# lhwright13/Hybrid-Classical-and-Reinforcement-Learning-Aircraft-Controllers

Hardware: AMD Instinct MI355X
Metric: env-steps/sec (whole node), rate-control task, batch 65536 per GPU (higher is better)
Workload: dtype f32 compute / f64 state

## Files before the change

hybrid-classical-and-reinforcement-learning-aircraft-controllers_amd/csrc/fdyn_core.hpp:

```cpp
#pragma once
#include <hip/hip_runtime.h>
#include <stdint.h>
#include "../../include/fdyn_layout.h"
#include "philox.hpp"

namespace fdyn {

#define FD_DEV __device__ __forceinline__

template <typename T> struct M;
template <> struct M<double> {
    static FD_DEV double sin(double x) { return ::sin(x); }
    static FD_DEV double cos(double x) { return ::cos(x); }
    static FD_DEV void sincos(double x, double& s, double& c) { ::sincos(x, &s, &c); }
    static FD_DEV double tan(double x) { return ::tan(x); }
    static FD_DEV double atan2(double y, double x) { return ::atan2(y, x); }
    static FD_DEV double asin(double x) { return ::asin(x); }
    static FD_DEV double sqrt(double x) { return ::sqrt(x); }
    static FD_DEV double exp(double x) { return ::exp(x); }
    static FD_DEV double abs(double x) { return ::fabs(x); }
    static FD_DEV double copysign(double a, double y) { return __builtin_copysign(a, y); }
    static FD_DEV double rint(double x) { return ::rint(x); }
    static FD_DEV double fmod(double x, double y) { return ::fmod(x, y); }
    static FD_DEV bool finite(double x) { return ::isfinite(x); }
// ... 26 lines not shown
FD_DEV f32x2 pk_fma(f32x2 a, f32x2 b, f32x2 c) { return __builtin_elementwise_fma(a, b, c); }
FD_DEV f32x2 bc(float x) { return (f32x2){ x, x }; }
FD_DEV f32x2 lo_only(float x) { f32x2 r; r.x = x; return r; }
FD_DEV f32x2 pk_fma_bx_nhi(f32x2 a, f32x2 b, f32x2 c)
{
    f32x2 d;
    asm("v_pk_fma_f32 %0, %1, %2, %3 op_sel_hi:[1,0,1] neg_hi:[0,0,1]" : "=v"(d) : "v"(a), "v"(b), "v"(c));
    return d;
}
FD_DEV f32x2 pk_fma_ayx_bx_nlo(f32x2 a, f32x2 b, f32x2 c)
{
    f32x2 d;
    asm("v_pk_fma_f32 %0, %1, %2, %3 op_sel:[1,0,0] op_sel_hi:[0,0,1] neg_lo:[0,0,1]" : "=v"(d) : "v"(a), "v"(b), "v"(c));
    return d;
}
FD_DEV f32x2 rotate_small(f32x2 sc, float d)
{
    const float z = d * d;
    const f32x2 p1 = pk_fma(bc(z), (f32x2){ 4.1666667908e-2f, 8.3333337680e-3f }, (f32x2){ -0.5f, -1.6666667163e-1f });
    const f32x2 p2 = pk_fma(bc(z), p1, (f32x2){ 1.0f, 0.0f });
    const float sd = __builtin_fmaf(p2.y, d, d);
    return pk_fma_bx_nhi(sc, p2, sc.yx * bc(sd));
}
FD_DEV float cos_bounded(float x)
{
    const float z = x * x;
    float p = __builtin_fmaf(z, 2.4801587e-5f, -1.3888889e-3f);
    p = __builtin_fmaf(z, p, 4.1666668e-2f);
    p = __builtin_fmaf(z, p, -0.5f);
    float c = __builtin_fmaf(z, p, 1.0f);
    if (__builtin_expect(!(z <= 0.64f), 0)) { float sn; sincos(x, sn, c); }
    return c;
}
#define FD_ATAN_WIDE_LIMIT 0.7f
FD_DEV float atan_wide(float t)
{
    const float z = t * t;
    float p = __builtin_fmaf(z, 2.0541535690e-02f, -6.1546623707e-02f);
    p = __builtin_fmaf(z, p, 1.0221967846e-01f);
    p = __builtin_fmaf(z, p, -1.4136675000e-01f);
    p = __builtin_fmaf(z, p, 1.9987617433e-01f);
    p = __builtin_fmaf(z, p, -3.3332955837e-01f);
    return __builtin_fmaf(p * z, t, t);
}
#define FD_ASIN_WIDE_LIMIT 0.75f
FD_DEV float asin_wide(float x)
// ... 6 lines not shown
    p = __builtin_fmaf(z, p, 4.1755288839e-02f);
    p = __builtin_fmaf(z, p, 7.5183674693e-02f);
    p = __builtin_fmaf(z, p, 1.6666238010e-01f);
    return __builtin_fmaf(p * z, x, x);
}
FD_DEV float asin_wide_t(float t, float z)
{
    float p = __builtin_fmaf(z, 2.1202674508e-01f, -3.1944271922e-01f);
    p = __builtin_fmaf(z, p, 2.6334178448e-01f);
    p = __builtin_fmaf(z, p, -7.6388612390e-02f);
    p = __builtin_fmaf(z, p, 5.3024884313e-02f);
    p = __builtin_fmaf(z, p, 4.1755288839e-02f);
    p = __builtin_fmaf(z, p, 7.5183674693e-02f);
    p = __builtin_fmaf(z, p, 1.6666238010e-01f);
    return __builtin_fmaf(p * z, t, t);
}
FD_DEV f32x2 atan_asin_wide(float ta, float za, float tb, float zb)
{
    const float pa = __builtin_fmaf(za, 2.0541535690e-02f, -6.1546623707e-02f);
    float pb = __builtin_fmaf(zb, 2.1202674508e-01f, -3.1944271922e-01f);
    pb = __builtin_fmaf(zb, pb, 2.6334178448e-01f);
    pb = __builtin_fmaf(zb, pb, -7.6388612390e-02f);
    const f32x2 z = { za, zb }, t = { ta, tb };
    f32x2 p = pk_fma(z, (f32x2){ pa, pb }, (f32x2){ 1.0221967846e-01f, 5.3024884313e-02f });
    p = pk_fma(z, p, (f32x2){ -1.4136675000e-01f, 4.1755288839e-02f });
    p = pk_fma(z, p, (f32x2){ 1.9987617433e-01f, 7.5183674693e-02f });
    p = pk_fma(z, p, (f32x2){ -3.3332955837e-01f, 1.6666238010e-01f });
    return pk_fma(p * z, t, t);
}
FD_DEV float atan_pos(float a)
{
    const bool big = a > 2.414213562373095f, mid = a > 0.4142135623730950f;
    const float num = big ? -1.0f : (mid ? a - 1.0f : a);
    const float den = big ? a : (mid ? a + 1.0f : 1.0f);
    const float base = big ? 1.5707963267948966f : (mid ? 0.7853981633974483f : 0.0f);
    const float t = num * rcp(den);
    const float z = t * t;
    float p = __builtin_fmaf(z, 8.05374449538e-2f, -1.38776856032e-1f);
    p = __builtin_fmaf(z, p, 1.99777106478e-1f);
    p = __builtin_fmaf(z, p, -3.33329491539e-1f);
    return base + __builtin_fmaf(p * z, t, t);
}
FD_DEV float atan2(float y, float x)
{
    const float ax = __builtin_fabsf(x), ay = __builtin_fabsf(y);
    const float mx = __builtin_fmaxf(ax, ay), mn = __builtin_fminf(ax, ay);
// ... 137 lines not shown
        derive_lane_from<FAST>(lane, src[derive_source(lane < FD_ND_LANES ? lane : 0)], blk);
    }
    template <bool FAST>
    static FD_DEV void derive_lane_from(int lane, double a, double* blk)
    {
        if (lane < 5) {
            const int to = lane == 0 ? FD_PD_INV_MASS : (lane == 1 ? FD_PD_INV_IXX : (lane == 2 ? FD_PD_INV_IYY : (lane == 3 ? FD_PD_INV_IZZ : FD_PD_INV_THRUST_ZERO_V)));
            blk[to] = 1.0 / a;
        } else if (FAST && lane < FD_ND_LANES) {
            const bool is_alpha = lane == 5;
            float snf, csf;
            fast::sincos(float(a), snf, csf);
            const double sn = snf, cs = csf;
            blk[is_alpha ? FD_PD_SIN_MAX_ALPHA : FD_PD_SIN_MAX_PITCH] = sn;
            blk[is_alpha ? FD_PD_COS_MAX_ALPHA : FD_PD_COS_MAX_PITCH] = cs;
            if (is_alpha) {
                const double tl = sn / cs;
                const bool poly_ok = a > 0.0 && a < 1.5 && tl <= double(FD_ATAN_WIDE_LIMIT);
                blk[FD_PD_TAN_ALPHA_FAST] = poly_ok ? tl : 0.0;
                blk[FD_PD_ALPHA_NEEDS_ATAN2] = poly_ok ? 0.0 : 1.0;
            }
        }
    }
};

template <typename S> struct Limits {
    S max_vel, max_rate, max_pitch, min_dt, max_dt;
    FD_DEV void load(const double* blk)
    {
        max_vel = S(blk[FD_P_MAX_VELOCITY]); max_rate = S(blk[FD_P_MAX_RATE_RAD]);
        max_pitch = S(blk[FD_P_MAX_PITCH_RAD]); min_dt = S(blk[FD_P_MIN_TIMESTEP]); max_dt = S(blk[FD_P_MAX_TIMESTEP]);
    }
};

template <typename T> struct Controls {
    T de_rad, da_rad, dr_rad, throttle;
    T cl0_de, cm_de, cl_da, cn_dr, cy, thrust_max;
    fast::f32x2 pk_da_dr;
    template <typename S> FD_DEV void set(const Params<T>& P, S elevator, S aileron, S rudder, S thr)
    {
        de_rad = T(clipv<S>(elevator, S(-1), S(1))) * P.max_de;
        da_rad = T(clipv<S>(aileron, S(-1), S(1))) * P.max_da;
        dr_rad = T(clipv<S>(rudder, S(-1), S(1))) * P.max_dr;
        throttle = T(clipv<S>(thr, S(0), S(1)));
        if constexpr (sizeof(T) == 4) {
            cl0_de = P.cl_0 + P.cl_de * de_rad;
// ... 122 lines not shown
struct Trig { fast::f32x2 phi, th, psi; };
FD_DEV Trig trig_of(float phi, float theta, float psi)
{
    Trig t;
    float s, c;
    fast::sincos(phi, s, c); t.phi = (fast::f32x2){ s, c };
    fast::sincos(theta, s, c); t.th = (fast::f32x2){ s, c };
    fast::sincos(psi, s, c); t.psi = (fast::f32x2){ s, c };
    return t;
}
FD_DEV float trig_rotate(const Trig& t0, float dphi, float dth, float dpsi, Trig& t)
{
    t.phi = fast::rotate_small(t0.phi, dphi);
    t.th = fast::rotate_small(t0.th, dth);
    t.psi = fast::rotate_small(t0.psi, dpsi);
    return __builtin_fmaxf(__builtin_fmaxf(__builtin_fabsf(dphi), __builtin_fabsf(dth)), __builtin_fabsf(dpsi));
}
FD_DEV float trig_rotate_scaled(const Trig& t0, float h, float kphi, float kth, float kpsi, Trig& t)
{
    const fast::f32x2 d2 = fast::bc(h) * (fast::f32x2){ kphi, kth };
    return trig_rotate(t0, d2.x, d2.y, h * kpsi, t);
}

#define FD_UNLIKELY(c) __builtin_expect(!!(c), 0)
#ifdef FD_PHASE_STAMPS
__device__ unsigned fdyn_dbg_cnt[4096 * 8];
#define FD_DBG_COUNT(SLOT) if (threadIdx.x < 64) { const unsigned long long m_ = __ballot(1); \
    if (int(threadIdx.x) == __ffsll((long long)m_) - 1) atomicAdd(&fdyn_dbg_cnt[blockIdx.x * 8 + (SLOT)], 1u); \
    atomicAdd(&fdyn_dbg_cnt[blockIdx.x * 8 + (SLOT) + 1], 1u); }
#define FD_DBG_COUNT1(SLOT) if (threadIdx.x < 64) atomicAdd(&fdyn_dbg_cnt[blockIdx.x * 8 + (SLOT)], 1u);
#else
#define FD_DBG_COUNT(SLOT)
#define FD_DBG_COUNT1(SLOT)
#endif

template <bool STRAIGHT = true, bool WIND = false>
FD_DEV void dynamics_fast(const Params<float>& P, const Controls<float>& C, const float (&x)[FD_NX], Trig& tg, float dmax,
                          float (&xd)[FD_NX], const Wind<float>& wnd = Wind<float>{})
{
    const float ug = x[3], vg = x[4], wg = x[5], theta = x[7];
    const float p = x[9], q = x[10], r = x[11];
    float u = ug, v = vg, w = wg;
    if constexpr (WIND) {
        if (FD_UNLIKELY(!(dmax <= 0.125f))) { tg = trig_of(x[6], theta, x[8]); dmax = 0.0f; }
        float bu, bv, bw;
        body_wind<float>(tg.phi.x, tg.phi.y, tg.th.x, tg.th.y, tg.psi.x, tg.psi.y, wnd, bu, bv, bw);
        u = ug - bu; v = vg - bv; w = wg - bw;
    }

    const fast::f32x2 vw = { v, w };
    const fast::f32x2 vw_sq = vw * vw;
    const float uw2 = __builtin_fmaf(u, u, vw_sq.y);
    const float V2 = __builtin_fmaf(v, v, uw2);
    const float airspeed = fast::sqrt(V2);
    const float Vs = fast::max_nc(airspeed, P.min_airspeed);
    const float inv_V = fast::rcp(Vs);

    const float au = __builtin_fabsf(u);
    const float au_min = fast::max_nc(au, P.min_u);
    const float us = au > 1e-6f ? __builtin_copysignf(au_min, u) : P.min_u;
    const float inv_h = fast::rsq(__builtin_fmaf(us, us, vw_sq.y));
    const fast::f32x2 xt_ab = vw * (fast::f32x2){ inv_V, fast::rcp(us) };
    const fast::f32x2 xt_sq = xt_ab * xt_ab;
    const float t_alpha = xt_ab.y;
    const bool a_in = __builtin_fabsf(w) <= P.tan_alpha_fast * us;
    const float sin_alpha = a_in ? w * inv_h : __builtin_copysignf(P.sin_max_alpha, w);
    const float cos_alpha = a_in ? us * inv_h : P.cos_max_alpha;

    const float av = __builtin_fabsf(v);
    const bool b_in = av <= FD_ASIN_WIDE_LIMIT * Vs;
    const float xb = xt_ab.x;
    auto beta_tail = [&]() {
        const float vv_rest = airspeed >= P.min_airspeed ? uw2 : __builtin_fmaxf(__builtin_fmaf(Vs, Vs, -(v * v)), 0.0f);
        const float half_om = 0.5f * (vv_rest * fast::rcp(Vs * (Vs + av)));
        const float b_r = fast::asin_wide_t(fast::sqrt(half_om), half_om);
        return __builtin_copysignf(__builtin_fmaf(-2.0f, b_r, 1.5707963267948966f), v);
    };
    float beta, b_t, z_b;
    if constexpr (STRAIGHT) {
        const float vv_rest = airspeed >= P.min_airspeed ? uw2 : __builtin_fmaxf(__builtin_fmaf(Vs, Vs, -vw_sq.x), 0.0f);
        const float half_om = 0.5f * (vv_rest * fast::rcp(Vs * (Vs + av)));
        b_t = b_in ? xb : fast::sqrt(half_om);
        z_b = b_in ? xt_sq.x : half_om;
    } else {
        b_t = xb; z_b = xt_sq.x;
    }
    const fast::f32x2 ab = fast::atan_asin_wide(t_alpha, xt_sq.y, b_t, z_b);
    const float alpha_poly = fast::pinned(ab.x);
    const float alpha = a_in ? alpha_poly : __builtin_copysignf(P.max_alpha, w);
    if constexpr (STRAIGHT) beta = b_in ? ab.y : __builtin_copysignf(__builtin_fmaf(-2.0f, ab.y, 1.5707963267948966f), v);
    else beta = ab.y;

    const bool th_in = __builtin_fabsf(theta) <= P.max_pitch;
    float sth_e = th_in ? tg.th.x : __builtin_copysignf(P.sin_max_pitch, theta);
    float cth_e = th_in ? tg.th.y : P.cos_max_pitch;

    const bool ordinary = (dmax <= 0.125f) & (P.alpha_needs_atan2 == 0.0f) & (STRAIGHT | b_in);
    float alpha_r = alpha, sin_alpha_r = sin_alpha, cos_alpha_r = cos_alpha;
    if (FD_UNLIKELY(!ordinary)) {
        FD_DBG_COUNT(0)
        if (!(dmax <= 0.125f)) {
            FD_DBG_COUNT1(4)
            tg = trig_of(x[6], theta, x[8]);
            sth_e = th_in ? tg.th.x : sth_e; cth_e = th_in ? tg.th.y : cth_e;
        }
        if (P.alpha_needs_atan2 != 0.0f) {
            const float a_raw = fast::atan2(w, us);
            const bool hi = a_raw > P.max_alpha, lo = a_raw < -P.max_alpha;
            sin_alpha_r = hi ? P.sin_max_alpha : (lo ? -P.sin_max_alpha : w * inv_h);
            cos_alpha_r = (hi || lo) ? P.cos_max_alpha : us * inv_h;
            alpha_r = clipf(a_raw, -P.max_alpha, P.max_alpha);
        }
        if constexpr (!STRAIGHT) {
            if (!b_in) beta = beta_tail();
        }
    }
    const float sth = tg.th.x, cth = tg.th.y;

    using fast::f32x2;
    using fast::bc;
    const float q_S = P.half_rho_S * V2;
    const float cl = __builtin_fmaf(P.cl_alpha, alpha_r, C.cl0_de);
    const float cd = __builtin_fmaf(P.cd_alpha2, alpha_r * alpha_r, P.cd_0);
    const f32x2 ld = bc(q_S) * (f32x2){ cl, cd };
    const f32x2 cs_a = { cos_alpha_r, sin_alpha_r };
    const f32x2 fxz = fast::pk_fma_ayx_bx_nlo(cs_a, ld, ld.yy * cs_a);
    const float thrust = C.thrust_max * __builtin_fmaxf(0.0f, __builtin_fmaf(-airspeed, P.inv_thrust_zero_v, 1.0f));

    const f32x2 g_cs = bc(P.g) * (tg.phi * bc(cth));
    xd[3] = __builtin_fmaf(fxz.x + thrust, P.inv_mass, __builtin_fmaf(r, vg, __builtin_fmaf(-q, wg, -(P.g * sth))));
    xd[4] = __builtin_fmaf(q_S * C.cy, P.inv_mass, __builtin_fmaf(p, wg, __builtin_fmaf(-r, ug, g_cs.x)));
    xd[5] = __builtin_fmaf(-fxz.y, P.inv_mass, __builtin_fmaf(q, ug, __builtin_fmaf(-p, vg, g_cs.y)));

    const f32x2 hV = P.pk_half_b_c * bc(inv_V);
    const f32x2 qSbc = bc(q_S) * P.pk_b_c;
    const f32x2 pr = { p, r };
    const f32x2 ln_in = fast::pk_fma(P.pk_damp_pr * pr, bc(hV.x), C.pk_da_dr);
    const f32x2 ln = bc(qSbc.x) * fast::pk_fma(P.pk_beta_ln, bc(beta), ln_in);
    const float m_moment = qSbc.y * __builtin_fmaf(P.cm_alpha, alpha_r, __builtin_fmaf(P.damp_pitch * q, hV.y, C.cm_de));
    const f32x2 gy = { __builtin_fmaf(-P.izz_m_iyy * q, r, ln.x), __builtin_fmaf(-P.iyy_m_ixx * p, q, ln.y) };
    const f32x2 a_pr = gy * P.pk_inv_i_pr;
    xd[9] = a_pr.x;
    xd[10] = __builtin_fmaf(-P.ixx_m_izz * p, r, m_moment) * P.inv_iyy;
    xd[11] = a_pr.y;

    const fast::f32x2 sb = fast::pk_fma_bx_nhi(tg.phi, fast::lo_only(vg), tg.phi.yx * fast::bc(wg));
    const float sv_cw = sb.x;
    const float ah = __builtin_fmaf(cth, ug, sth * sv_cw);
    const fast::f32x2 ne = fast::pk_fma_ayx_bx_nlo(tg.psi, fast::lo_only(ah), tg.psi * fast::bc(sb.y));
    xd[0] = ne.x;
    xd[1] = ne.y;
    xd[2] = __builtin_fmaf(cth, sv_cw, -(sth * ug));

    const float inv_c = fast::rcp(cth_e);
    const fast::f32x2 qt = fast::pk_fma_bx_nhi(tg.phi, fast::lo_only(q), tg.phi.yx * fast::bc(r));
    const float qr = qt.x;
    xd[8] = qr * inv_c;
    xd[6] = __builtin_fmaf(sth_e * inv_c, qr, p);
    xd[7] = qt.y;

#pragma unroll
    for (int i = 9; i < 12; ++i) xd[i] = clipf(xd[i], -P.max_ang_acc, P.max_ang_acc);
// ... 20 lines not shown
        const S v = x[i];
        x[i] = (v != v) ? S(0) : (M<S>::finite(v) ? v : (v > S(0) ? S(10000) : S(-10000)));
    }
#pragma unroll
    for (int i = 3; i < 6; ++i) x[i] = clipv(x[i], -Lm.max_vel, Lm.max_vel);
    x[6] = wrap_state_angle<S, T>(x[6]);
    x[7] = clipv(x[7], -Lm.max_pitch, Lm.max_pitch);
    x[8] = wrap_state_angle<S, T>(x[8]);
#pragma unroll
    for (int i = 9; i < 12; ++i) x[i] = clipv(x[i], -Lm.max_rate, Lm.max_rate);
    if (-x[2] < S(0)) {
        x[2] = S(0);
        x[5] = x[5] > S(0) ? x[5] : S(0);
    }
    S accs = x[0];
#pragma unroll
    for (int i = 1; i < 12; ++i) accs += x[i];
    if (!M<S>::finite(accs)) {
#pragma unroll
        for (int i = 0; i < 12; ++i) x[i] = M<S>::finite(x[i]) ? x[i] : S(0);
    }
}

struct FastRK {
    float x0[FD_NX];
    Trig t0;
    float d0;
    template <typename S> FD_DEV void init(const S (&x)[FD_NX])
    {
#pragma unroll
        for (int i = 0; i < 12; ++i) x0[i] = float(x[i]);
        t0 = trig_of(x0[6], x0[7], x0[8]);
        d0 = 0.0f;
    }
    FD_DEV void ensure_trig()
    {
        if (FD_UNLIKELY(!(d0 <= 0.125f))) { t0 = trig_of(x0[6], x0[7], x0[8]); d0 = 0.0f; }
    }
};

template <typename S, bool STRAIGHT = true, bool WIND = false>
FD_DEV void rk4_fast_step(const Params<float>& P, const Limits<S>& Lm, const Controls<float>& C, S (&x)[FD_NX], FastRK& f,
                          float hdt, float fdt, float dt6, const Wind<float>& wnd = Wind<float>{})
{
    using T = float;
    T xt[FD_NX], k[FD_NX];
    Trig tt;
    using fast::f32x2;
    constexpr int PA[6] = { 0, 2, 4, 6, 8, 10 }, PB[6] = { 1, 3, 5, 7, 9, 11 };
    f32x2 acc2[6], x02[6];
#pragma unroll
    for (int j = 0; j < 6; ++j) x02[j] = (f32x2){ f.x0[PA[j]], f.x0[PB[j]] };
    auto stage = [&](T h, T wgt, bool first) {
#pragma unroll
        for (int j = 0; j < 6; ++j) {
            const f32x2 kj = { k[PA[j]], k[PB[j]] };
            acc2[j] = first ? kj : fast::pk_fma(fast::bc(wgt), kj, acc2[j]);
            if (j >= 1) {
                const f32x2 xj = fast::pk_fma(fast::bc(h), kj, x02[j]);
                xt[PA[j]] = xj.x; xt[PB[j]] = xj.y;
            }
        }
    };
    dynamics_fast<STRAIGHT, WIND>(P, C, f.x0, f.t0, f.d0, k, wnd);
    stage(hdt, T(1), true);
    T dm = trig_rotate_scaled(f.t0, hdt, k[6], k[7], k[8], tt);
    dynamics_fast<STRAIGHT, WIND>(P, C, xt, tt, dm, k, wnd);
    stage(hdt, T(2), false);
    dm = trig_rotate_scaled(f.t0, hdt, k[6], k[7], k[8], tt);
    dynamics_fast<STRAIGHT, WIND>(P, C, xt, tt, dm, k, wnd);
    stage(fdt, T(2), false);
    dm = trig_rotate_scaled(f.t0, fdt, k[6], k[7], k[8], tt);
    dynamics_fast<STRAIGHT, WIND>(P, C, xt, tt, dm, k, wnd);
    T ksum[FD_NX], inc[FD_NX];
#pragma unroll
    for (int j = 0; j < 6; ++j) {
        const f32x2 ks = acc2[j] + (f32x2){ k[PA[j]], k[PB[j]] };
        const f32x2 in2 = fast::bc(dt6) * ks;
        ksum[PA[j]] = ks.x; ksum[PB[j]] = ks.y;
        inc[PA[j]] = in2.x; inc[PB[j]] = in2.y;
    }
#pragma unroll
    for (int i = 0; i < 12; ++i) {
        if constexpr (sizeof(S) == 4) x[i] = __builtin_fmaf(dt6, ksum[i], x[i]);
        else x[i] += S(inc[i]);
        if (STRAIGHT && i >= 9) x[i] = M<S>::abs(x[i]) > Lm.max_rate ? M<S>::copysign(Lm.max_rate, x[i]) : x[i];
        f.x0[i] = T(x[i]);
    }
    f.d0 = trig_rotate(f.t0, inc[6], inc[7], inc[8], f.t0);
    f32x2 sum2 = { f.x0[0], f.x0[1] };
#pragma unroll
    for (int j = 1; j < 6; ++j) sum2 += (f32x2){ f.x0[2 * j], f.x0[2 * j + 1] };
    const T sum = sum2.x + sum2.y;
    const T vmax = __builtin_fmaxf(__builtin_fmaxf(__builtin_fabsf(f.x0[3]), __builtin_fabsf(f.x0[4])), __builtin_fabsf(f.x0[5]));
    const T amax = __builtin_fmaxf(__builtin_fabsf(f.x0[6]), __builtin_fabsf(f.x0[8]));
    bool lim = !(vmax <= T(Lm.max_vel)) | (f.x0[2] > T(0)) | !(amax <= T(FD_PI));
    if constexpr (!STRAIGHT) {
        lim |= (M<S>::abs(x[9]) > Lm.max_rate) | (M<S>::abs(x[10]) > Lm.max_rate) | (M<S>::abs(x[11]) > Lm.max_rate);
    }
    const bool ang = !(__builtin_fabsf(f.x0[7]) <= T(Lm.max_pitch)) | !M<T>::finite(sum);
    if (FD_UNLIKELY(lim | ang)) {
        FD_DBG_COUNT(2)
#ifdef FD_PHASE_STAMPS
        if (!(vmax <= T(Lm.max_vel))) { FD_DBG_COUNT1(5) }
        if (f.x0[2] > T(0)) { FD_DBG_COUNT1(7) }
#endif
        if (ang) {
            post_step<S, T>(Lm, x);
#pragma unroll
            for (int i = 0; i < 12; ++i) f.x0[i] = T(x[i]);
            f.d0 = T(1);
        } else {
#pragma unroll
            for (int i = 3; i < 6; ++i) x[i] = clipv(x[i], -Lm.max_vel, Lm.max_vel);
            if constexpr (!STRAIGHT) {
#pragma unroll
                for (int i = 9; i < 12; ++i) {
                    x[i] = M<S>::abs(x[i]) > Lm.max_rate ? M<S>::copysign(Lm.max_rate, x[i]) : x[i];
                    f.x0[i] = T(x[i]);
                }
            }
            x[6] = wrap_state_angle<S, T>(x[6]);
            x[8] = wrap_state_angle<S, T>(x[8]);
            if (-x[2] < S(0)) {
                x[2] = S(0);
                x[5] = x[5] > S(0) ? x[5] : S(0);
            }
            f.x0[2] = T(x[2]); f.x0[6] = T(x[6]); f.x0[8] = T(x[8]);
#pragma unroll
            for (int i = 3; i < 6; ++i) f.x0[i] = T(x[i]);
        }
    }
}

template <typename S, typename T, bool STRAIGHT = true, bool WIND = false>
FD_DEV void rk4_substeps(const Params<T>& P, const Limits<S>& Lm, const Controls<T>& C, S (&x)[FD_NX], S dt, int n_sub,
                         const Wind<T>& wnd = Wind<T>{})
{
    if constexpr (sizeof(T) == 8) {
        for (int s = 0; s < n_sub; ++s) {
            T xt[FD_NX], k[FD_NX];
            S acc[FD_NX];
            const T hdt = T(S(0.5) * dt), fdt = T(dt);
#pragma unroll
            for (int i = 0; i < 12; ++i) xt[i] = T(x[i]);
            dynamics<T, WIND>(P, C, xt, k, wnd);
#pragma unroll
            for (int i = 0; i < 12; ++i) { acc[i] = S(k[i]); xt[i] = T(x[i] + S(hdt) * S(k[i])); }
            dynamics<T, WIND>(P, C, xt, k, wnd);
#pragma unroll
            for (int i = 0; i < 12; ++i) { acc[i] += S(2) * S(k[i]); xt[i] = T(x[i] + S(hdt) * S(k[i])); }
            dynamics<T, WIND>(P, C, xt, k, wnd);
#pragma unroll
            for (int i = 0; i < 12; ++i) { acc[i] += S(2) * S(k[i]); xt[i] = T(x[i] + S(fdt) * S(k[i])); }
            dynamics<T, WIND>(P, C, xt, k, wnd);
            const S dt6 = dt / S(6);
#pragma unroll
            for (int i = 0; i < 12; ++i) x[i] = x[i] + dt6 * (acc[i] + S(k[i]));
            post_step<S, T>(Lm, x);
        }
    } else {
        FastRK f;
        f.init(x);
        const T hdt = T(S(0.5) * dt), fdt = T(dt), dt6 = T(dt / S(6));
        for (int s = 0; s < n_sub; ++s) rk4_fast_step<S, STRAIGHT, WIND>(P, Lm, C, x, f, hdt, fdt, dt6, wnd);
    }
}

template <typename S> struct Derived { S airspeed, altitude, ground_speed, heading; };
template <typename S> FD_DEV Derived<S> derived(const S (&x)[FD_NX])
{
    Derived<S> d;
    const S u = x[3], v = x[4], w = x[5];
    S sphi, cphi, sth, cth, spsi, cpsi;
    M<S>::sincos(x[6], sphi, cphi);
    M<S>::sincos(x[7], sth, cth);
    M<S>::sincos(x[8], spsi, cpsi);
    d.airspeed = M<S>::sqrt(u * u + v * v + w * w);
    d.altitude = -x[2];
    const S vn = (cth * cpsi) * u + (sphi * sth * cpsi - cphi * spsi) * v + (cphi * sth * cpsi + sphi * spsi) * w;
    const S ve = (cth * spsi) * u + (sphi * sth * spsi + cphi * cpsi) * v + (cphi * sth * spsi - sphi * cpsi) * w;
    d.heading = M<S>::atan2(ve, vn);
    d.ground_speed = M<S>::sqrt(vn * vn + ve * ve);
    return d;
}
FD_DEV Derived<float> derived_fast(FastRK& f)
{
    f.ensure_trig();
// ... 301 lines not shown
```

hybrid-classical-and-reinforcement-learning-aircraft-controllers_amd/csrc/fdyn_kernels.hip:

```cpp
#include <hip/hip_runtime.h>
#include <stdint.h>
#include <math.h>
#include <string.h>
#include <stdlib.h>
#include "fdyn_fleet.hpp"

using namespace fdyn;

#define FD_BLOCK 256

struct StagedParamWords { double v0, v1, d; };
__device__ __forceinline__ StagedParamWords stage_params_early(const double* __restrict__ params, int n_types)
{
    StagedParamWords w;
    const int i0 = threadIdx.x, i1 = FD_BLOCK + threadIdx.x;
    const int t0 = i0 / FD_NP_USED, t1 = i1 / FD_NP_USED;
    w.v0 = i0 < n_types * FD_NP_USED ? params[t0 * FD_NP + (i0 - t0 * FD_NP_USED)] : 0.0;
    w.v1 = i1 < n_types * FD_NP_USED ? params[t1 * FD_NP + (i1 - t1 * FD_NP_USED)] : 0.0;
    constexpr int NDL = Params<double>::FD_ND_LANES;
    const int t = threadIdx.x / NDL;
    w.d = int(threadIdx.x) < n_types * NDL ? params[t * FD_NP + Params<double>::derive_source(threadIdx.x - t * NDL)] : 1.0;
    return w;
}
template <bool FAST>
// ... 812 lines not shown
                     const double* __restrict__ pool, int pool_depth, uint64_t seed, int auto_reset, float residual_scale,
                     float* __restrict__ obs_out , float* __restrict__ reward_f32, S* __restrict__ reward_full,
                     uint8_t* __restrict__ terminated, uint8_t* __restrict__ truncated,
                     int32_t* __restrict__ ev_count, int32_t* __restrict__ ev_count_next, int32_t* __restrict__ ev_int,
                     float* __restrict__ ev_flt, int ev_cap, int64_t n, DRA... dra)
{
    constexpr bool DR = sizeof...(DRA) != 0;
    S* dr = nullptr;
    const double* drc = nullptr;
    if constexpr (DR) dr_unpack(dr, drc, dra...);
    __shared__ double s_params[FD_MAX_TYPES * FD_NP_STAGED];
    __shared__ __attribute__((aligned(16))) float s_tile[FD_BLOCK / FD_WAVE][FD_WAVE * (FD_OBS_DIM + 1)];
    __shared__ float s_pid_cfg[3 * FD_NPC];
    __shared__ S s_consts[FD_NC];
    FD_STAMP(0)
    FD_STAMP_REAL(7)
    const LaneMap lm = lane_map(n);
    const int64_t i = lm.i;
    const int lane = lm.lane, wave = threadIdx.x / FD_WAVE;
    const bool active = lm.on;
    EnvConsts<S> ec;
    load_env_consts<S, PREP>(EC, ec);
    const bool uses_sched = ec.cmd_type == FD_CMD_RAMP || ec.cmd_type == FD_CMD_SINE;
    const bool residual_mode = actions != nullptr && residual_scale > 0.0f && pid_state != nullptr;
    const bool pid_mode = actions == nullptr || residual_mode;

    using E = typename EnvOf<S, T>::type;
    S x[FD_NX];
    EnvState<E> e;
    int32_t step = 0, episode = 0;
    int ty = 0;
    float4 av = make_float4(0.0f, 0.0f, 0.0f, 0.0f);
    S rec_pre[FD_NR];
    S wair[3] = { S(0), S(0), S(0) }, dsc[5] = { S(1), S(1), S(1), S(1), S(1) };
    const bool pre_drawn = !OCC2 && pool == nullptr && auto_reset != 0;
    constexpr bool EARLY_PARAMS = sizeof(T) == 4;
    StagedParamWords spw = { 0.0, 0.0, 1.0 };
    if constexpr (EARLY_PARAMS) spw = PREP ? stage_image_early(params, n_types) : stage_params_early(params, n_types);
    if (active) {
        episode = eis[FD_EI_EPISODE * n + i];
#pragma unroll
        for (int k = 3; k < FD_NX; ++k) x[k] = xs[k * n + i];
        if (actions) av = reinterpret_cast<const float4*>(actions)[i];
        ty = lane_type(type, i, n_types);
#pragma unroll
        for (int k = 0; k < 3; ++k) x[k] = xs[k * n + i];
// ... 57 lines not shown
#pragma unroll
                for (int k = 0; k < 4; ++k) {
                    const float c = a_in[k] + rr[k] * residual_scale;
                    const float lo = k < 3 ? -1.0f : 0.0f;
                    a_in[k] = c < lo ? lo : (c > 1.0f ? 1.0f : c);
                }
                const float mag = rr[0] * rr[0] + (rr[1] * rr[1] + rr[2] * rr[2]);
                res_bonus = S(0.05) * (S(1) - S(mag) / S(3));
            }
        }
        if (actions_out) reinterpret_cast<float4*>(actions_out)[i] = make_float4(a_in[0], a_in[1], a_in[2], a_in[3]);
        S a[4];
        a[0] = clipv(S(a_in[0]), S(-1), S(1)); a[1] = clipv(S(a_in[1]), S(-1), S(1));
        a[2] = clipv(S(a_in[2]), S(-1), S(1)); a[3] = clipv(S(a_in[3]), S(0), S(1));

        Controls<T> C;
        C.set(P, a[1], a[0], a[2], a[3]);
        const S dt_sub = ec.dt / S(ec.n_sub);
#ifdef FD_PHASE_STAMPS
        asm volatile("s_waitcnt vmcnt(0) lgkmcnt(0)" ::: "memory");
#endif
        FD_STAMP(1)
        if constexpr (DR) rk4_substeps<S, T, !OCC2, true>(P, Lm, C, x, dt_sub, ec.n_sub, Wind<T>{ T(wair[0]), T(wair[1]), T(wair[2]) });
        else rk4_substeps<S, T, !OCC2>(P, Lm, C, x, dt_sub, ec.n_sub);
        FD_STAMP(2)
        if constexpr (sizeof(E) == sizeof(S)) e.time += E(ec.dt);
        else e.time = E(S(step + 1) * ec.dt);
        step += 1;

        if (ec.cmd_type == FD_CMD_RAMP) {
            const S t = S(e.time);
            if (t < S(3)) {
                const S alpha = t / S(3);
#pragma unroll
                for (int k = 0; k < 3; ++k) e.cmd[k] = E((S(1) - alpha) * S(0) + alpha * S(e.sched[k]));
            } else {
#pragma unroll
                for (int k = 0; k < 3; ++k) e.cmd[k] = e.sched[k];
            }
        } else if (ec.cmd_type == FD_CMD_RANDOM_WALK) {
            S delta[3];
            if (rw_delta) {
#pragma unroll
                for (int k = 0; k < 3; ++k) delta[k] = rw_delta[k * n + i];
            } else {
                Philox ph; uint32_t r[4];
                ph.block(seed, uint32_t(i), uint32_t(episode), uint32_t(step), FD_PHX_RANDOM_WALK, r);
// ... 101 lines not shown
            const int leader = __ffsll((long long)done_mask) - 1;
            base = __shfl(base, leader, FD_WAVE);
            const int local = base + prefix;
            if (done && local < cap_s) {
                const int slot = shard * cap_s + local;
                ev_int[slot * FD_EV_NI + FD_EV_ENV] = int32_t(i);
                ev_int[slot * FD_EV_NI + FD_EV_LENGTH] = len_term;
                ev_int[slot * FD_EV_NI + FD_EV_TERMINATED] = term ? 1 : 0;
                ev_flt[slot * FD_EV_NF] = ret_term;
#pragma unroll
                for (int k = 0; k < FD_OBS_DIM; ++k) ev_flt[slot * FD_EV_NF + 1 + k] = o_term[k];
            }
        }
    }
    FD_STAMP(4)
    store_obs_tile(s_tile[wave], o, lane, obs_out, lm.wave_first, n);
    FD_STAMP(5)
#ifdef FD_PHASE_STAMPS
    asm volatile("s_waitcnt vmcnt(0)" ::: "memory");
#endif
    FD_STAMP_REAL(6)
}

static_assert(FD_NIMG == FD_IMG_PARAMS + FD_MAX_TYPES * FD_NP_STAGED && FD_ECD_INTS + 2 <= FD_IMG_PARAMS, "fdyn_layout.h: image sections");
template <bool FAST>
__global__ void __launch_bounds__(FD_BLOCK)
rate_env_image_kernel(const double* __restrict__ params, int n_types, const double* __restrict__ EC, double* __restrict__ image)
{
    double* blocks = image + FD_IMG_PARAMS;
    for (int i = threadIdx.x; i < FD_MAX_TYPES * FD_NP_STAGED; i += blockDim.x) {
        const int t = i / FD_NP_STAGED, k = i - t * FD_NP_STAGED;
        blocks[i] = (t < n_types && k < FD_NP_USED) ? params[t * FD_NP + k] : 0.0;
    }
    for (int k = threadIdx.x; k < FD_IMG_PARAMS; k += blockDim.x) if (k < FD_ECD_INTS || k >= FD_ECD_INTS + 2) image[FD_IMG_EC + k] = k < FD_NEC ? EC[k] : 0.0;
    __syncthreads();
    constexpr int NDL = Params<double>::FD_ND_LANES;
    if (int(threadIdx.x) < n_types * NDL) {
        const int t = threadIdx.x / NDL;
        Params<double>::derive_lane<FAST>(threadIdx.x - t * NDL, params + t * FD_NP, blocks + t * FD_NP_STAGED);
    }
    if (threadIdx.x == FD_BLOCK - 1) {
        EnvConsts<double> ec;
        load_env_consts<double>(EC, ec);
        int32_t* ic = reinterpret_cast<int32_t*>(image + FD_IMG_EC + FD_ECD_INTS);
        ic[0] = ec.max_steps; ic[1] = ec.cmd_type; ic[2] = ec.n_sub; ic[3] = ec.settle_steps;
    }
}

static int g_simds = 0;
static int simd_count()
{
    if (!g_simds) {
        int dev = 0; hipDeviceProp_t p;
        g_simds = (hipGetDevice(&dev) == hipSuccess && hipGetDeviceProperties(&p, dev) == hipSuccess) ? p.multiProcessorCount * 4 : 1024;
    }
    return g_simds;
}

#define FD_ENV_RESET_PARAMS(S, E)                                                                            \
    S* x, E* e, int32_t* ei, float* pid_state, const uint8_t* mask, const double* env_consts, const double* pool, \
    int pool_depth, uint64_t seed, float* obs_out, int64_t n
#define FD_ENV_RESET_ARGS x, e, ei, pid_state, mask, env_consts, pool, pool_depth, seed, obs_out, n
#define FD_ENV_STEP_PARAMS(S, E)                                                                             \
    S* x, E* e, int32_t* ei, const uint8_t* type, const double* params, int n_types, const double* env_consts, \
    const float* actions, float* pid_state, const float* pid_cfg, const double* casc_consts, float* actions_out, \
    const S* rw_delta, const double* pool, int pool_depth, uint64_t seed, int auto_reset, float residual_scale, \
    float* obs_out, float* reward_f32, S* reward_full, uint8_t* terminated, uint8_t* truncated, int32_t* ev_count, \
    int32_t* ev_count_next, int32_t* ev_int, float* ev_flt, int ev_cap, int64_t n
// ... 193 lines not shown
```

include/fdyn_layout.h:

```cpp
#ifndef FDYN_LAYOUT_H
#define FDYN_LAYOUT_H

enum {
    FD_X_N = 0, FD_X_E, FD_X_D,
    FD_X_U, FD_X_V, FD_X_W,
    FD_X_ROLL, FD_X_PITCH, FD_X_YAW,
    FD_X_P, FD_X_Q, FD_X_R,
    FD_NX = 12
};

enum { FD_U_ELEVATOR = 0, FD_U_AILERON, FD_U_RUDDER, FD_U_THROTTLE, FD_NU = 4 };

enum { FD_D_AIRSPEED = 0, FD_D_ALTITUDE, FD_D_GROUND_SPEED, FD_D_HEADING, FD_ND = 4 };

enum {
    FD_P_MASS = 0, FD_P_IXX, FD_P_IYY, FD_P_IZZ,
    FD_P_WING_AREA, FD_P_WING_SPAN, FD_P_CHORD,
    FD_P_CL_0, FD_P_CL_ALPHA, FD_P_CD_0, FD_P_CD_ALPHA2,
    FD_P_CL_ELEVATOR, FD_P_CM_ELEVATOR, FD_P_CY_RUDDER, FD_P_CN_RUDDER, FD_P_CL_AILERON,
    FD_P_CM_ALPHA, FD_P_CN_BETA, FD_P_CL_BETA,
    FD_P_DAMPING_ROLL, FD_P_DAMPING_PITCH, FD_P_DAMPING_YAW,
    FD_P_MAX_THRUST, FD_P_AIR_DENSITY, FD_P_GRAVITY,
    FD_P_MIN_AIRSPEED_AERO, FD_P_MIN_U_VELOCITY,
    FD_P_MAX_ELEVATOR_RAD, FD_P_MAX_AILERON_RAD, FD_P_MAX_RUDDER_RAD,
// ... 44 lines not shown
enum { FD_CMD_STEP = 0, FD_CMD_RAMP = 1, FD_CMD_SINE = 2, FD_CMD_RANDOM_WALK = 3 };

enum {
    FD_E_CMD_P = 0, FD_E_CMD_Q, FD_E_CMD_R,
    FD_E_PREV_AIL, FD_E_PREV_ELEV, FD_E_PREV_RUD, FD_E_PREV_THR,
    FD_E_PERR_P, FD_E_PERR_Q, FD_E_PERR_R,
    FD_E_SIGN_P, FD_E_SIGN_Q, FD_E_SIGN_R,
    FD_E_SETTLE_TIMER, FD_E_IS_SETTLED,
    FD_E_TIME,
    FD_E_SCHED0, FD_E_SCHED1, FD_E_SCHED2,
    FD_E_SCHED3,
    FD_E_EP_RETURN,
    FD_NE = 21
};
enum { FD_EI_STEP = 0, FD_EI_EPISODE, FD_NEI = 2 };

enum {
    FD_EC_DT = 0, FD_EC_DT_PHYSICS, FD_EC_MAX_STEPS, FD_EC_CMD_TYPE, FD_EC_DIFFICULTY_SCALE,
    FD_EC_MAX_RATE_P, FD_EC_MAX_RATE_Q, FD_EC_MAX_RATE_R,
    FD_NEC = 8
};

enum {
    FD_ECD_INTS = FD_NEC,
    FD_IMG_EC = 0, FD_IMG_PARAMS = 16,
    FD_NIMG = FD_IMG_PARAMS + 8 * FD_NP_STAGED
};

enum {
    FD_R_AIRSPEED = 0, FD_R_ALTITUDE, FD_R_ROLL, FD_R_PITCH, FD_R_YAW, FD_R_P, FD_R_Q, FD_R_R,
    FD_R_CMD0, FD_R_CMD1, FD_R_CMD2,
    FD_R_CMD3,
    FD_NR = 12
};

enum { FD_EV_ENV = 0, FD_EV_LENGTH, FD_EV_TERMINATED, FD_EV_NI = 3 };
#define FD_EV_NF (1 + FD_OBS_DIM)
enum { FD_EV_SHARDS = 64 };

enum {
    FD_DR_WIND_N = 0, FD_DR_WIND_E, FD_DR_WIND_D,
    FD_DR_GUST_N, FD_DR_GUST_E, FD_DR_GUST_D,
    FD_DR_GUST_A, FD_DR_GUST_B,
    FD_DR_MASS_S, FD_DR_IXX_S, FD_DR_IYY_S, FD_DR_IZZ_S, FD_DR_RHO_S,
    FD_NDR = 13
};
enum {
// ... 92 lines not shown
```

Before: 1.779 billion.

## Add branch-free RK4 fast path when step-size bounds prove rare cases impossible

Computes, when the parameter image is built, an a priori bound on Euler-angle increments per substep. If every aircraft type satisfies it and the alpha polynomial is valid, a flag is stored in the image. The rate kernel then ballots whether any lane is outside the rate/pitch limits and, if none are, runs an RK4 variant with the rare-case checks (dmax, atan2 fallback, pinned values) compiled out. That variant also packs the trig rotation and damping arithmetic into paired f32 ops and keeps predicate literals in scalar registers. It adds a second instantiation of the substep loop, which costs code size and register pressure, and its correctness depends on the analytic bound holding.

Measured after the change: 1.871 billion, median of 6. 5.2% higher.

```diff
diff --git a/hybrid-classical-and-reinforcement-learning-aircraft-controllers_amd/csrc/fdyn_core.hpp b/hybrid-classical-and-reinforcement-learning-aircraft-controllers_amd/csrc/fdyn_core.hpp
--- a/hybrid-classical-and-reinforcement-learning-aircraft-controllers_amd/csrc/fdyn_core.hpp
+++ b/hybrid-classical-and-reinforcement-learning-aircraft-controllers_amd/csrc/fdyn_core.hpp
@@ -72,6 +72,14 @@
     const float sd = __builtin_fmaf(p2.y, d, d);
     return pk_fma_bx_nhi(sc, p2, sc.yx * bc(sd));
 }
+FD_DEV f32x2 rotate_small_bc(f32x2 sc, f32x2 dd)
+{
+    const float z = dd.x * dd.x;
+    const f32x2 p1 = pk_fma(bc(z), (f32x2){ 4.1666667908e-2f, 8.3333337680e-3f }, (f32x2){ -0.5f, -1.6666667163e-1f });
+    const f32x2 p2 = pk_fma(bc(z), p1, (f32x2){ 1.0f, 0.0f });
+    const f32x2 sd = pk_fma(p2.yy, dd, dd);
+    return pk_fma_bx_nhi(sc, p2, sc.yx * sd);
+}
 FD_DEV float cos_bounded(float x)
 {
     const float z = x * x;
@@ -124,6 +132,18 @@
     pb = __builtin_fmaf(zb, pb, 2.6334178448e-01f);
     pb = __builtin_fmaf(zb, pb, -7.6388612390e-02f);
     const f32x2 z = { za, zb }, t = { ta, tb };
+    f32x2 p = pk_fma(z, (f32x2){ pa, pb }, (f32x2){ 1.0221967846e-01f, 5.3024884313e-02f });
+    p = pk_fma(z, p, (f32x2){ -1.4136675000e-01f, 4.1755288839e-02f });
+    p = pk_fma(z, p, (f32x2){ 1.9987617433e-01f, 7.5183674693e-02f });
+    p = pk_fma(z, p, (f32x2){ -3.3332955837e-01f, 1.6666238010e-01f });
+    return pk_fma(p * z, t, t);
+}
+FD_DEV f32x2 atan_asin_wide(f32x2 t, f32x2 z)
+{
+    const float pa = __builtin_fmaf(z.x, 2.0541535690e-02f, -6.1546623707e-02f);
+    float pb = __builtin_fmaf(z.y, 2.1202674508e-01f, -3.1944271922e-01f);
+    pb = __builtin_fmaf(z.y, pb, 2.6334178448e-01f);
+    pb = __builtin_fmaf(z.y, pb, -7.6388612390e-02f);
     f32x2 p = pk_fma(z, (f32x2){ pa, pb }, (f32x2){ 1.0221967846e-01f, 5.3024884313e-02f });
     p = pk_fma(z, p, (f32x2){ -1.4136675000e-01f, 4.1755288839e-02f });
     p = pk_fma(z, p, (f32x2){ 1.9987617433e-01f, 7.5183674693e-02f });
@@ -307,6 +327,16 @@
             }
         }
     }
+    static FD_DEV double euler_increment_bound(const double* __restrict__ src, double h)
+    {
+        constexpr double SLACK = 1.0 + 1.0 / 512.0;
+        const double R = src[FD_P_MAX_RATE_RAD], A = src[FD_P_MAX_ANGULAR_ACCELERATION], mp = src[FD_P_MAX_PITCH_RAD];
+        if (!(R >= 0.0 && A >= 0.0 && h > 0.0 && mp >= 0.0 && mp <= 1.5)) return 1.0e300;
+        const double rt2 = 1.4142135623730951;
+        const double G = fmax(1.0 + rt2 * tan(mp), rt2 / cos(mp));
+        return SLACK * h * G * (R + 0.5 * h * A);
+    }
+    static FD_DEV bool small_steps_ok(const double* __restrict__ src, double h) { return euler_increment_bound(src, h) <= 0.125; }
 };
 
 template <typename S> struct Limits {
@@ -475,6 +505,13 @@
     return trig_rotate(t0, d2.x, d2.y, h * kpsi, t);
 }
 
+FD_DEV void trig_rotate_pairs(const Trig& t0, fast::f32x2 d2, fast::f32x2 dpsi, Trig& t)
+{
+    t.phi = fast::rotate_small_bc(t0.phi, d2.xx);
+    t.th = fast::rotate_small_bc(t0.th, d2.yy);
+    t.psi = fast::rotate_small_bc(t0.psi, dpsi.xx);
+}
+
 #define FD_UNLIKELY(c) __builtin_expect(!!(c), 0)
 #ifdef FD_PHASE_STAMPS
 __device__ unsigned fdyn_dbg_cnt[4096 * 8];
@@ -487,10 +524,11 @@
 #define FD_DBG_COUNT1(SLOT)
 #endif
 
-template <bool STRAIGHT = true, bool WIND = false>
+template <bool STRAIGHT = true, bool WIND = false, bool RARE = true>
 FD_DEV void dynamics_fast(const Params<float>& P, const Controls<float>& C, const float (&x)[FD_NX], Trig& tg, float dmax,
                           float (&xd)[FD_NX], const Wind<float>& wnd = Wind<float>{})
 {
+    static_assert(RARE || (STRAIGHT && !WIND), "the block-free form exists for the straight, still-air evaluation only");
     const float ug = x[3], vg = x[4], wg = x[5], theta = x[7];
     const float p = x[9], q = x[10], r = x[11];
     float u = ug, v = vg, w = wg;
@@ -513,16 +551,23 @@
     const float au_min = fast::max_nc(au, P.min_u);
     const float us = au > 1e-6f ? __builtin_copysignf(au_min, u) : P.min_u;
     const float inv_h = fast::rsq(__builtin_fmaf(us, us, vw_sq.y));
-    const fast::f32x2 xt_ab = vw * (fast::f32x2){ inv_V, fast::rcp(us) };
+    constexpr int IA = RARE ? 1 : 0, IB = 1 - IA;
+    fast::f32x2 xt_ab, rcps = { 0.0f, 0.0f };
+    if constexpr (RARE) xt_ab = vw * (fast::f32x2){ inv_V, fast::rcp(us) };
+    else {
+        rcps = (fast::f32x2){ fast::rcp(us), inv_V };
+        asm("" : "+v"(rcps));
+        xt_ab = vw.yx * rcps;
+    }
     const fast::f32x2 xt_sq = xt_ab * xt_ab;
-    const float t_alpha = xt_ab.y;
+    const float t_alpha = xt_ab[IA];
     const bool a_in = __builtin_fabsf(w) <= P.tan_alpha_fast * us;
     const float sin_alpha = a_in ? w * inv_h : __builtin_copysignf(P.sin_max_alpha, w);
     const float cos_alpha = a_in ? us * inv_h : P.cos_max_alpha;
 
     const float av = __builtin_fabsf(v);
     const bool b_in = av <= FD_ASIN_WIDE_LIMIT * Vs;
-    const float xb = xt_ab.x;
+    const float xb = xt_ab[IB];
     auto beta_tail = [&]() {
         const float vv_rest = airspeed >= P.min_airspeed ? uw2 : __builtin_fmaxf(__builtin_fmaf(Vs, Vs, -(v * v)), 0.0f);
         const float half_om = 0.5f * (vv_rest * fast::rcp(Vs * (Vs + av)));
@@ -534,12 +579,20 @@
         const float vv_rest = airspeed >= P.min_airspeed ? uw2 : __builtin_fmaxf(__builtin_fmaf(Vs, Vs, -vw_sq.x), 0.0f);
         const float half_om = 0.5f * (vv_rest * fast::rcp(Vs * (Vs + av)));
         b_t = b_in ? xb : fast::sqrt(half_om);
-        z_b = b_in ? xt_sq.x : half_om;
+        z_b = b_in ? xt_sq[IB] : half_om;
     } else {
-        b_t = xb; z_b = xt_sq.x;
-    }
-    const fast::f32x2 ab = fast::atan_asin_wide(t_alpha, xt_sq.y, b_t, z_b);
-    const float alpha_poly = fast::pinned(ab.x);
+        b_t = xb; z_b = xt_sq[IB];
+    }
+    fast::f32x2 ab;
+    if constexpr (RARE) {
+        ab = fast::atan_asin_wide(t_alpha, xt_sq[IA], b_t, z_b);
+    } else {
+        fast::f32x2 t2 = xt_ab, z2 = xt_sq;
+        t2.y = b_t; z2.y = z_b;
+        ab = fast::atan_asin_wide(t2, z2);
+    }
+    float alpha_poly = ab.x;
+    if constexpr (RARE) alpha_poly = fast::pinned(ab.x);
     const float alpha = a_in ? alpha_poly : __builtin_copysignf(P.max_alpha, w);
     if constexpr (STRAIGHT) beta = b_in ? ab.y : __builtin_copysignf(__builtin_fmaf(-2.0f, ab.y, 1.5707963267948966f), v);
     else beta = ab.y;
@@ -548,7 +601,7 @@
     float sth_e = th_in ? tg.th.x : __builtin_copysignf(P.sin_max_pitch, theta);
     float cth_e = th_in ? tg.th.y : P.cos_max_pitch;
 
-    const bool ordinary = (dmax <= 0.125f) & (P.alpha_needs_atan2 == 0.0f) & (STRAIGHT | b_in);
+    const bool ordinary = RARE ? (dmax <= 0.125f) & (P.alpha_needs_atan2 == 0.0f) & (STRAIGHT | b_in) : true;
     float alpha_r = alpha, sin_alpha_r = sin_alpha, cos_alpha_r = cos_alpha;
     if (FD_UNLIKELY(!ordinary)) {
         FD_DBG_COUNT(0)
@@ -580,17 +633,30 @@
     const f32x2 fxz = fast::pk_fma_ayx_bx_nlo(cs_a, ld, ld.yy * cs_a);
     const float thrust = C.thrust_max * __builtin_fmaxf(0.0f, __builtin_fmaf(-airspeed, P.inv_thrust_zero_v, 1.0f));
 
-    const f32x2 g_cs = bc(P.g) * (tg.phi * bc(cth));
+    f32x2 g_cs;
+    if constexpr (RARE) g_cs = bc(P.g) * (tg.phi * bc(cth));
+    else g_cs = bc(P.g) * (tg.phi * tg.th.yy);
     xd[3] = __builtin_fmaf(fxz.x + thrust, P.inv_mass, __builtin_fmaf(r, vg, __builtin_fmaf(-q, wg, -(P.g * sth))));
     xd[4] = __builtin_fmaf(q_S * C.cy, P.inv_mass, __builtin_fmaf(p, wg, __builtin_fmaf(-r, ug, g_cs.x)));
     xd[5] = __builtin_fmaf(-fxz.y, P.inv_mass, __builtin_fmaf(q, ug, __builtin_fmaf(-p, vg, g_cs.y)));
 
-    const f32x2 hV = P.pk_half_b_c * bc(inv_V);
+    f32x2 hV;
+    if constexpr (RARE) hV = P.pk_half_b_c * bc(inv_V);
+    else hV = P.pk_half_b_c * rcps.yy;
     const f32x2 qSbc = bc(q_S) * P.pk_b_c;
-    const f32x2 pr = { p, r };
-    const f32x2 ln_in = fast::pk_fma(P.pk_damp_pr * pr, bc(hV.x), C.pk_da_dr);
+    f32x2 ln_in;
+    float damp_q = 0.0f;
+    if constexpr (RARE) {
+        const f32x2 pr = { p, r };
+        ln_in = fast::pk_fma(P.pk_damp_pr * pr, bc(hV.x), C.pk_da_dr);
+    } else {
+        const f32x2 d_qr = (f32x2){ P.damp_pitch, P.pk_damp_pr.y } * (f32x2){ q, r };
+        ln_in = (f32x2){ __builtin_fmaf(P.pk_damp_pr.x * p, hV.x, C.pk_da_dr.x), __builtin_fmaf(d_qr.y, hV.x, C.pk_da_dr.y) };
+        damp_q = d_qr.x;
+    }
     const f32x2 ln = bc(qSbc.x) * fast::pk_fma(P.pk_beta_ln, bc(beta), ln_in);
-    const float m_moment = qSbc.y * __builtin_fmaf(P.cm_alpha, alpha_r, __builtin_fmaf(P.damp_pitch * q, hV.y, C.cm_de));
+    if constexpr (RARE) damp_q = P.damp_pitch * q;
+    const float m_moment = qSbc.y * __builtin_fmaf(P.cm_alpha, alpha_r, __builtin_fmaf(damp_q, hV.y, C.cm_de));
     const f32x2 gy = { __builtin_fmaf(-P.izz_m_iyy * q, r, ln.x), __builtin_fmaf(-P.iyy_m_ixx * p, q, ln.y) };
     const f32x2 a_pr = gy * P.pk_inv_i_pr;
     xd[9] = a_pr.x;
@@ -657,10 +723,13 @@
     }
 }
 
+struct PredLits { float pi, inf, zero; };
 struct FastRK {
     float x0[FD_NX];
     Trig t0;
     float d0;
+    fast::f32x2 xp[FD_NX / 2];
+    PredLits lit;
     template <typename S> FD_DEV void init(const S (&x)[FD_NX])
     {
 #pragma unroll
@@ -674,11 +743,19 @@
     }
 };
 
-template <typename S, bool STRAIGHT = true, bool WIND = false>
+template <typename S, bool STRAIGHT = true, bool WIND = false, bool RARE = true>
 FD_DEV void rk4_fast_step(const Params<float>& P, const Limits<S>& Lm, const Controls<float>& C, S (&x)[FD_NX], FastRK& f,
                           float hdt, float fdt, float dt6, const Wind<float>& wnd = Wind<float>{})
 {
     using T = float;
+    if constexpr (!RARE) {
+#pragma unroll
+        for (int j = 0; j < 6; ++j) {
+            fast::f32x2 v = f.xp[j];
+            asm("" : "+v"(v));
+            f.x0[2 * j] = v.x; f.x0[2 * j + 1] = v.y;
+        }
+    }
     T xt[FD_NX], k[FD_NX];
     Trig tt;
     using fast::f32x2;
@@ -697,16 +774,23 @@
             }
         }
     };
-    dynamics_fast<STRAIGHT, WIND>(P, C, f.x0, f.t0, f.d0, k, wnd);
+    dynamics_fast<STRAIGHT, WIND, RARE>(P, C, f.x0, f.t0, f.d0, k, wnd);
     stage(hdt, T(1), true);
-    T dm = trig_rotate_scaled(f.t0, hdt, k[6], k[7], k[8], tt);
-    dynamics_fast<STRAIGHT, WIND>(P, C, xt, tt, dm, k, wnd);
+    auto rotate_stage = [&](T h) {
+        trig_rotate_pairs(f.t0, fast::bc(h) * (f32x2){ k[6], k[7] }, fast::bc(h) * (f32x2){ k[8], k[9] }, tt);
+    };
+    T dm = T(0);
+    if constexpr (RARE) dm = trig_rotate_scaled(f.t0, hdt, k[6], k[7], k[8], tt);
+    else rotate_stage(hdt);
+    dynamics_fast<STRAIGHT, WIND, RARE>(P, C, xt, tt, dm, k, wnd);
     stage(hdt, T(2), false);
-    dm = trig_rotate_scaled(f.t0, hdt, k[6], k[7], k[8], tt);
-    dynamics_fast<STRAIGHT, WIND>(P, C, xt, tt, dm, k, wnd);
+    if constexpr (RARE) dm = trig_rotate_scaled(f.t0, hdt, k[6], k[7], k[8], tt);
+    else rotate_stage(hdt);
+    dynamics_fast<STRAIGHT, WIND, RARE>(P, C, xt, tt, dm, k, wnd);
     stage(fdt, T(2), false);
-    dm = trig_rotate_scaled(f.t0, fdt, k[6], k[7], k[8], tt);
-    dynamics_fast<STRAIGHT, WIND>(P, C, xt, tt, dm, k, wnd);
+    if constexpr (RARE) dm = trig_rotate_scaled(f.t0, fdt, k[6], k[7], k[8], tt);
+    else rotate_stage(fdt);
+    dynamics_fast<STRAIGHT, WIND, RARE>(P, C, xt, tt, dm, k, wnd);
     T ksum[FD_NX], inc[FD_NX];
 #pragma unroll
     for (int j = 0; j < 6; ++j) {
@@ -722,18 +806,23 @@
         if (STRAIGHT && i >= 9) x[i] = M<S>::abs(x[i]) > Lm.max_rate ? M<S>::copysign(Lm.max_rate, x[i]) : x[i];
         f.x0[i] = T(x[i]);
     }
-    f.d0 = trig_rotate(f.t0, inc[6], inc[7], inc[8], f.t0);
+    if constexpr (RARE) f.d0 = trig_rotate(f.t0, inc[6], inc[7], inc[8], f.t0);
+    else trig_rotate_pairs(f.t0, (f32x2){ inc[6], inc[7] }, (f32x2){ inc[8], inc[9] }, f.t0);
     f32x2 sum2 = { f.x0[0], f.x0[1] };
 #pragma unroll
     for (int j = 1; j < 6; ++j) sum2 += (f32x2){ f.x0[2 * j], f.x0[2 * j + 1] };
     const T sum = sum2.x + sum2.y;
     const T vmax = __builtin_fmaxf(__builtin_fmaxf(__builtin_fabsf(f.x0[3]), __builtin_fabsf(f.x0[4])), __builtin_fabsf(f.x0[5]));
     const T amax = __builtin_fmaxf(__builtin_fabsf(f.x0[6]), __builtin_fabsf(f.x0[8]));
-    bool lim = !(vmax <= T(Lm.max_vel)) | (f.x0[2] > T(0)) | !(amax <= T(FD_PI));
+    bool lim;
+    if constexpr (RARE) lim = !(vmax <= T(Lm.max_vel)) | (f.x0[2] > T(0)) | !(amax <= T(FD_PI));
+    else lim = !(vmax <= T(Lm.max_vel)) | (f.x0[2] > f.lit.zero) | !(amax <= f.lit.pi);
     if constexpr (!STRAIGHT) {
         lim |= (M<S>::abs(x[9]) > Lm.max_rate) | (M<S>::abs(x[10]) > Lm.max_rate) | (M<S>::abs(x[11]) > Lm.max_rate);
     }
-    const bool ang = !(__builtin_fabsf(f.x0[7]) <= T(Lm.max_pitch)) | !M<T>::finite(sum);
+    bool ang;
+    if constexpr (RARE) ang = !(__builtin_fabsf(f.x0[7]) <= T(Lm.max_pitch)) | !M<T>::finite(sum);
+    else ang = !(__builtin_fabsf(f.x0[7]) <= T(Lm.max_pitch)) | !(__builtin_fabsf(sum) < f.lit.inf);
     if (FD_UNLIKELY(lim | ang)) {
         FD_DBG_COUNT(2)
 #ifdef FD_PHASE_STAMPS
@@ -744,7 +833,12 @@
             post_step<S, T>(Lm, x);
 #pragma unroll
             for (int i = 0; i < 12; ++i) f.x0[i] = T(x[i]);
-            f.d0 = T(1);
+            if constexpr (RARE) {
+                f.d0 = T(1);
+            } else {
+                f.t0 = trig_of(f.x0[6], f.x0[7], f.x0[8]);
+                f.d0 = T(0);
+            }
         } else {
 #pragma unroll
             for (int i = 3; i < 6; ++i) x[i] = clipv(x[i], -Lm.max_vel, Lm.max_vel);
@@ -766,9 +860,13 @@
             for (int i = 3; i < 6; ++i) f.x0[i] = T(x[i]);
         }
     }
-}
-
-template <typename S, typename T, bool STRAIGHT = true, bool WIND = false>
+    if constexpr (!RARE) {
+#pragma unroll
+        for (int j = 0; j < 6; ++j) f.xp[j] = (f32x2){ f.x0[2 * j], f.x0[2 * j + 1] };
+    }
+}
+
+template <typename S, typename T, bool STRAIGHT = true, bool WIND = false, bool RARE = true>
 FD_DEV void rk4_substeps(const Params<T>& P, const Limits<S>& Lm, const Controls<T>& C, S (&x)[FD_NX], S dt, int n_sub,
                          const Wind<T>& wnd = Wind<T>{})
 {
@@ -798,7 +896,15 @@
         FastRK f;
         f.init(x);
         const T hdt = T(S(0.5) * dt), fdt = T(dt), dt6 = T(dt / S(6));
-        for (int s = 0; s < n_sub; ++s) rk4_fast_step<S, STRAIGHT, WIND>(P, Lm, C, x, f, hdt, fdt, dt6, wnd);
+        if constexpr (RARE) {
+            for (int s = 0; s < n_sub; ++s) rk4_fast_step<S, STRAIGHT, WIND, RARE>(P, Lm, C, x, f, hdt, fdt, dt6, wnd);
+        } else {
+#pragma unroll
+            for (int j = 0; j < 6; ++j) f.xp[j] = (fast::f32x2){ f.x0[2 * j], f.x0[2 * j + 1] };
+            f.lit = PredLits{ float(FD_PI), __builtin_inff(), 0.0f };
+            asm volatile("" : "+s"(f.lit.pi), "+s"(f.lit.inf), "+s"(f.lit.zero));
+            for (int s = 0; s < n_sub; ++s) rk4_fast_step<S, STRAIGHT, WIND, RARE>(P, Lm, C, x, f, hdt, fdt, dt6, wnd);
+        }
     }
 }
 
diff --git a/hybrid-classical-and-reinforcement-learning-aircraft-controllers_amd/csrc/fdyn_kernels.hip b/hybrid-classical-and-reinforcement-learning-aircraft-controllers_amd/csrc/fdyn_kernels.hip
--- a/hybrid-classical-and-reinforcement-learning-aircraft-controllers_amd/csrc/fdyn_kernels.hip
+++ b/hybrid-classical-and-reinforcement-learning-aircraft-controllers_amd/csrc/fdyn_kernels.hip
@@ -858,6 +858,9 @@
     EnvConsts<S> ec;
     load_env_consts<S, PREP>(EC, ec);
     const bool uses_sched = ec.cmd_type == FD_CMD_RAMP || ec.cmd_type == FD_CMD_SINE;
+    constexpr bool TWO_LOOPS = PREP && !OCC2 && !DR && sizeof(S) == 8 && sizeof(T) == 4;
+    bool small_steps = false;
+    if constexpr (TWO_LOOPS) small_steps = EC[FD_ECD_SMALL_STEPS] != 0.0;
     const bool residual_mode = actions != nullptr && residual_scale > 0.0f && pid_state != nullptr;
     const bool pid_mode = actions == nullptr || residual_mode;
 
@@ -961,7 +964,14 @@
 #endif
         FD_STAMP(1)
         if constexpr (DR) rk4_substeps<S, T, !OCC2, true>(P, Lm, C, x, dt_sub, ec.n_sub, Wind<T>{ T(wair[0]), T(wair[1]), T(wair[2]) });
-        else rk4_substeps<S, T, !OCC2>(P, Lm, C, x, dt_sub, ec.n_sub);
+        else if constexpr (TWO_LOOPS) {
+            const float r_max = float(Lm.max_rate), p_max = float(Lm.max_pitch);
+            const bool outside = !(__builtin_fabsf(float(x[9])) <= r_max) | !(__builtin_fabsf(float(x[10])) <= r_max) |
+                                 !(__builtin_fabsf(float(x[11])) <= r_max) | !(__builtin_fabsf(float(x[7])) <= p_max) |
+                                 !(__builtin_fabsf(float(x[6])) < __builtin_inff()) | !(__builtin_fabsf(float(x[8])) < __builtin_inff());
+            if (small_steps && __ballot(outside) == 0ull) rk4_substeps<S, T, true, false, false>(P, Lm, C, x, dt_sub, ec.n_sub);
+            else rk4_substeps<S, T, true>(P, Lm, C, x, dt_sub, ec.n_sub);
+        } else rk4_substeps<S, T, !OCC2>(P, Lm, C, x, dt_sub, ec.n_sub);
         FD_STAMP(2)
         if constexpr (sizeof(E) == sizeof(S)) e.time += E(ec.dt);
         else e.time = E(S(step + 1) * ec.dt);
@@ -1109,7 +1119,8 @@
     FD_STAMP_REAL(6)
 }
 
-static_assert(FD_NIMG == FD_IMG_PARAMS + FD_MAX_TYPES * FD_NP_STAGED && FD_ECD_INTS + 2 <= FD_IMG_PARAMS, "fdyn_layout.h: image sections");
+static_assert(FD_NIMG == FD_IMG_PARAMS + FD_MAX_TYPES * FD_NP_STAGED && FD_ECD_INTS + 2 <= FD_ECD_SMALL_STEPS &&
+              FD_ECD_SMALL_STEPS < FD_IMG_PARAMS, "fdyn_layout.h: image sections");
 template <bool FAST>
 __global__ void __launch_bounds__(FD_BLOCK)
 rate_env_image_kernel(const double* __restrict__ params, int n_types, const double* __restrict__ EC, double* __restrict__ image)
@@ -1119,7 +1130,7 @@
         const int t = i / FD_NP_STAGED, k = i - t * FD_NP_STAGED;
         blocks[i] = (t < n_types && k < FD_NP_USED) ? params[t * FD_NP + k] : 0.0;
     }
-    for (int k = threadIdx.x; k < FD_IMG_PARAMS; k += blockDim.x) if (k < FD_ECD_INTS || k >= FD_ECD_INTS + 2) image[FD_IMG_EC + k] = k < FD_NEC ? EC[k] : 0.0;
+    for (int k = threadIdx.x; k < FD_IMG_PARAMS; k += blockDim.x) if ((k < FD_ECD_INTS || k >= FD_ECD_INTS + 2) && k != FD_ECD_SMALL_STEPS) image[FD_IMG_EC + k] = k < FD_NEC ? EC[k] : 0.0;
     __syncthreads();
     constexpr int NDL = Params<double>::FD_ND_LANES;
     if (int(threadIdx.x) < n_types * NDL) {
@@ -1131,6 +1142,19 @@
         load_env_consts<double>(EC, ec);
         int32_t* ic = reinterpret_cast<int32_t*>(image + FD_IMG_EC + FD_ECD_INTS);
         ic[0] = ec.max_steps; ic[1] = ec.cmd_type; ic[2] = ec.n_sub; ic[3] = ec.settle_steps;
+        bool small = FAST;
+        if constexpr (FAST) {
+            const double dt_sub = ec.dt / double(ec.n_sub);
+            for (int t = 0; t < n_types; ++t) {
+                const double* src = params + t * FD_NP;
+                const double a = src[FD_P_MAX_ALPHA_RAD];
+                float snf, csf;
+                fast::sincos(float(a), snf, csf);
+                const bool poly_ok = a > 0.0 && a < 1.5 && double(snf) / double(csf) <= double(FD_ATAN_WIDE_LIMIT);
+                small = small && poly_ok && Params<double>::small_steps_ok(src, dt_sub);
+            }
+        }
+        image[FD_IMG_EC + FD_ECD_SMALL_STEPS] = small ? 1.0 : 0.0;
     }
 }
 
diff --git a/include/fdyn_layout.h b/include/fdyn_layout.h
--- a/include/fdyn_layout.h
+++ b/include/fdyn_layout.h
@@ -90,7 +90,7 @@
 };
 
 enum {
-    FD_ECD_INTS = FD_NEC,
+    FD_ECD_INTS = FD_NEC, FD_ECD_SMALL_STEPS = FD_NEC + 2,
     FD_IMG_EC = 0, FD_IMG_PARAMS = 16,
     FD_NIMG = FD_IMG_PARAMS + 8 * FD_NP_STAGED
 };
```
